# ChalmersPhotonicsLab/QAMpy

Hardware: AMD Instinct MI355X
Metric: equalised MSym/s (2-pol, 2 SPS) (higher is better)
Workload: dtype f32

## Files before the change

### qampy_amd/csrc/api.hip

```cpp
#include "common.h"
#include <stdlib.h>
#include <atomic>
#include <mutex>
#include <vector>
#include <unordered_map>
#include <string.h>

namespace qh {

thread_local hipStream_t g_stream = nullptr;
static thread_local hipStream_t g_streams[4] = {nullptr, nullptr, nullptr, nullptr};
int g_device = -1;
static thread_local std::string g_err;
static std::mutex g_mu;

void set_error(const std::string &s) { g_err = s; }

int hip_fail(hipError_t e, const char *what, const char *file, int line)
{
    g_err = std::string(hipGetErrorString(e)) + " in " + what + " (" + file + ":" + std::to_string(line) + ")";
    (void)hipGetLastError();
    return QH_ERR_HIP;
}

// ... 4 lines not shown
static int reserved_cus()
{
    int v = g_reserved_cus.load();
    if (v < 0) { const char *e = getenv("QAMPY_HIP_RESERVED_CUS"); v = e ? atoi(e) : 32; if (v < 0) v = 0; g_reserved_cus.store(v); }
    return v;
}
double gram_budget_gb()
{
    double v = g_gram_budget_gb.load();
    if (v < 0) { const char *e = getenv("QAMPY_HIP_GRAM_BUDGET_GB"); v = e ? atof(e) : 160.0; if (!(v > 0)) v = 160.0; g_gram_budget_gb.store(v); }
    return v;
}
static std::atomic<int> g_pit_timing{-1};
int pit_timing_mode()
{
    int v = g_pit_timing.load();
    if (v < 0) { const char *e = getenv("QAMPY_HIP_PIT_TIMING"); v = !e ? 1 : (e[0] == 'a' ? 2 : (e[0] == 'n' ? 0 : 1)); g_pit_timing.store(v); }
    return v;
}
int default_tier() { return g_default_tier.load(); }
double default_tier_tol() { return g_default_tol.load(); }

static int init_device(int device)
{
    std::lock_guard<std::mutex> lk(g_mu);
    if (g_stream && device == g_device) return QH_OK;
    if (g_device >= 0 && device != g_device) {
        set_error("libqampy_hip is already initialised on device " + std::to_string(g_device) + ": one device per process");
        return QH_ERR_ARG;
    }
    int n = 0;
    if (hipGetDeviceCount(&n) != hipSuccess || n <= 0) {
        (void)hipGetLastError();
        set_error("no HIP device visible: libqampy_hip needs a gfx950 (MI355X) GPU, there is no CPU fallback");
        return QH_ERR_NODEVICE;
    }
    if (device < 0 || device >= n) { set_error("device index out of range"); return QH_ERR_ARG; }
    hipDeviceProp_t prop;
    QH_HIP(hipGetDeviceProperties(&prop, device));
    if (strncmp(prop.gcnArchName, "gfx950", 6) != 0) {
        set_error(std::string("device is ") + prop.gcnArchName + ", libqampy_hip is built for gfx950 only");
        return QH_ERR_NODEVICE;
    }
    QH_HIP(hipSetDevice(device));
    int prio_least = 0, prio_greatest = 0;
    QH_HIP(hipDeviceGetStreamPriorityRange(&prio_least, &prio_greatest));
    for (int i = 0; i < 4; i++) {
        if (g_streams[i]) { (void)hipStreamDestroy(g_streams[i]); g_streams[i] = nullptr; }
        if (i == 2) {
            const int reserved = reserved_cus();
            const int ncu = prop.multiProcessorCount;
            if (reserved > 0 && reserved < ncu) {
                std::vector<uint32_t> mask((ncu + 31) / 32, 0u);
                for (int c = reserved; c < ncu; c++) mask[c / 32] |= 1u << (c % 32);
                if (hipExtStreamCreateWithCUMask(&g_streams[i], (uint32_t)mask.size(), mask.data()) == hipSuccess) continue;
                (void)hipGetLastError();
                g_streams[i] = nullptr;
            }
        }
        QH_HIP(hipStreamCreateWithPriority(&g_streams[i], hipStreamNonBlocking, i == 2 ? prio_least : prio_greatest));
    }
    g_stream = g_streams[0];
    g_device = device;
    return QH_OK;
}

hipStream_t side_stream() { return g_stream == g_streams[0] ? g_streams[1] : g_streams[0]; }
hipStream_t helper_stream() { return g_streams[3]; }

int ensure_init()
{
    if (g_stream) return QH_OK;
    return init_device(g_device >= 0 ? g_device : 0);
}

constexpr int SCRATCH_SLOTS = (int)Slot::COUNT;
thread_local void *g_scratch[SCRATCH_SLOTS] = {nullptr};
thread_local size_t g_scratch_n[SCRATCH_SLOTS] = {0};
thread_local unsigned g_scratch_epoch = 0;
static std::atomic<int> g_form[FORM_COUNT];
struct FormName { const char *key, *env; };
static const FormName FORM_NAMES[FORM_COUNT] = {
    {"trainer", "QAMPY_HIP_TRAINER"}, {"pit_form", "QAMPY_HIP_PIT_FORM"}, {"seg_lanes", "QAMPY_HIP_SEG_LANES"}, {"pit_probe", "QAMPY_HIP_PIT_PROBE"},
    {"bps", "QAMPY_HIP_BPS"}, {"pit_tail", "QAMPY_HIP_PIT_TAIL"}};
static int form_parse(int k, const char *v, int *out)
{
    if (!v || !v[0]) { *out = 0; return 0; }
    switch (k) {
    case FORM_TRAINER: *out = v[0] == 'd' ? 1 : (v[0] == 'l' ? 2 : (v[0] == 'i' ? 3 : (v[0] == 'a' || v[0] == '0' ? 0 : -1))); break;
    case FORM_PIT: *out = v[0] == 's' ? 1 : (v[0] == 'b' ? 2 : (v[0] == 'a' || v[0] == '0' ? 0 : -1)); break;
    case FORM_SEG_LANES: { const int n = atoi(v); *out = (n == 8 || n == 16 || n == 0) ? n : -1; break; }
    case FORM_BPS: *out = v[0] == 't' ? 1 : (v[0] == 'l' ? 2 : (v[0] == 'a' || v[0] == '0' ? 0 : -1)); break;
    case FORM_PIT_TAIL: *out = v[0] == 's' ? 1 : (v[0] == 'a' || v[0] == '0' ? 0 : -1); break;
    default: *out = atoi(v) != 0 ? 1 : 0; break;
    }
    return *out < 0 ? -1 : 0;
}
static const int g_form_env_read = [] {
    for (int k = 0; k < FORM_COUNT; k++) {
        int v = 0;
        if (form_parse(k, getenv(FORM_NAMES[k].env), &v) == 0) g_form[k].store(v);
    }
    return 0;
}();
int form(FormKey k) { return g_form[k].load(std::memory_order_relaxed); }
const char *trainer_force()
{
    switch (form(FORM_TRAINER)) {
    case 1: return "direct";
    case 2: return "lookahead";
    case 3: return "iterative";
    default: return "";
    }
}
static constexpr int POOL_CLASSES = 48, POOL_KEEP = 8;
static constexpr size_t POOL_BYTES = (size_t)24 << 30;
static std::vector<void *> g_pool[POOL_CLASSES];
static size_t g_pool_bytes = 0;
static void pool_release();
static int pool_class(size_t bytes) { int k = 8; while (((size_t)1 << k) < bytes && k < POOL_CLASSES - 1) k++; return k; }
int pool_alloc(size_t bytes, void **p, size_t *cap)
{
    const int k = pool_class(bytes);
    *cap = (size_t)1 << k;
    {
        std::lock_guard<std::mutex> lk(g_mu);
        if (!g_pool[k].empty()) { *p = g_pool[k].back(); g_pool[k].pop_back(); g_pool_bytes -= *cap; return QH_OK; }
    }
    hipError_t e = hipMalloc(p, *cap);
    if (e == hipErrorOutOfMemory) {
        (void)hipGetLastError();
        (void)hipDeviceSynchronize();
        pool_release();
        e = hipMalloc(p, *cap);
    }
    QH_HIP(e);
    return QH_OK;
}
void pool_free(void *p, size_t cap)
{
    const int k = pool_class(cap);
    {
        std::lock_guard<std::mutex> lk(g_mu);
        if ((int)g_pool[k].size() < POOL_KEEP && g_pool_bytes + cap <= POOL_BYTES) { g_pool[k].push_back(p); g_pool_bytes += cap; return; }
    }
    (void)hipFree(p);
}
static std::unordered_map<void *, size_t> g_dlive;
static void pool_release()
{
    std::lock_guard<std::mutex> lk(g_mu);
    for (auto &v : g_pool) { for (void *p : v) (void)hipFree(p); v.clear(); }
    g_pool_bytes = 0;
}

static std::vector<void *> g_hpool[POOL_CLASSES];
static size_t g_hpool_bytes = 0;
static constexpr size_t HPOOL_BYTES = (size_t)8 << 30;
static std::vector<std::pair<void *, size_t>> g_hlive;
int pinned_alloc(size_t bytes, void **p)
{
    const int k = pool_class(bytes ? bytes : 1);
    const size_t cap = (size_t)1 << k;
    {
        std::lock_guard<std::mutex> lk(g_mu);
        if (!g_hpool[k].empty()) { *p = g_hpool[k].back(); g_hpool[k].pop_back(); g_hpool_bytes -= cap; g_hlive.emplace_back(*p, cap); return QH_OK; }
    }
    QH_HIP(hipHostMalloc(p, cap, hipHostMallocDefault));
    std::lock_guard<std::mutex> lk(g_mu);
    g_hlive.emplace_back(*p, cap);
    return QH_OK;
}
int pinned_free(void *p)
{
    size_t cap = 0;
    {
// ... 311 lines not shown
```

### qampy_amd/csrc/common.h

```cpp
#pragma once
#include <hip/hip_runtime.h>
#include <stdint.h>
#include <string>
#include <vector>
#include "../../include/qampy_hip.h"

namespace qh {

extern thread_local hipStream_t g_stream;
extern int g_device;
void set_error(const std::string &s);
int hip_fail(hipError_t e, const char *what, const char *file, int line);

#define QH_HIP(call)                                                        \
    do {                                                                    \
        hipError_t _e = (call);                                             \
        if (_e != hipSuccess) return qh::hip_fail(_e, #call, __FILE__, __LINE__); \
    } while (0)

#define QH_REQUIRE(cond, msg)                                   \
    do {                                                        \
        if (!(cond)) { qh::set_error(msg); return QH_ERR_ARG; } \
    } while (0)

#define QH_WAVE_FIRST() __builtin_amdgcn_s_setprio(3)

int ensure_init();
hipStream_t side_stream();
hipStream_t helper_stream();
enum FormKey { FORM_TRAINER = 0, FORM_PIT, FORM_SEG_LANES, FORM_PIT_PROBE, FORM_BPS, FORM_PIT_TAIL, FORM_COUNT };
int form(FormKey k);
const char *trainer_force();
double gram_budget_gb();
int pit_timing_mode();
int default_tier();
double default_tier_tol();
enum class Slot : int {
    BPS_ANGLES,
    BPS_CHUNKS,
    BPS_ALPHABET,
    TWOSTAGE,
    STEP_SIZES,
    GRAM,
    BI_LEVELS,
    PIT_WORK,
    PIT_CTRL,
    PIT_COV,
    PIT_BASIS,
    PIT_ROTATIONS,
    PIT_ACQ,
    PIT_MODEL,
    SER,
    SYNTH,
    METRICS,
    SNR_EST,
    AWGN_MC,
    CD_TABLE,
    RESAMPLE_TABLE,
    ROW_MOMENTS,
    FOE,
    IMPAIR,
    PMD,
    TXRESP,
    SOS,
    CPR,
    FFT,
    IQ,
    SYNC,
    PEAK,
    PILOT,
    PRECOMP,
    BLIND,
    HYBRID,
    FIBRE,
    COUNT
};
int scratch(Slot slot, size_t bytes, void **p);
unsigned scratch_epoch();

struct TableCache {
    std::string key;
    std::vector<char> host;
    void *dev = nullptr;
    unsigned epoch = 0;
    template <typename F> int get(Slot slot, const std::string &k, size_t bytes, F fill, const void **tab)
    {
        void *p = nullptr;
        int rc;
        if (dev && key == k && epoch == scratch_epoch()) {
            if ((rc = scratch(slot, bytes, &p))) return rc;
            if (p == dev) { *tab = p; return QH_OK; }
        }
        if (dev) QH_HIP(hipDeviceSynchronize());
        dev = nullptr;
        if ((rc = scratch(slot, bytes, &p))) return rc;
        host.resize(bytes);
        fill(host.data());
        QH_HIP(hipMemcpyAsync(p, host.data(), bytes, hipMemcpyHostToDevice, g_stream));
        key = k; dev = p; epoch = scratch_epoch();
        *tab = p;
        return QH_OK;
    }
};
template <typename T> inline void key_add(std::string &k, const T &v) { k.append(reinterpret_cast<const char *>(&v), sizeof(T)); }

constexpr double QH_PI = 3.14159265358979323846, QH_TWO_PI = 2 * QH_PI;

inline size_t up256(size_t n) { return (n + 255) & ~(size_t)255; }
struct ScratchLayout {
    size_t total = 0;
    size_t take(size_t bytes) { const size_t o = total; total += up256(bytes); return o; }
};
template <typename K> int dyn_lds(K kernel, size_t bytes)
// ... 158 lines not shown
```

### qampy_amd/csrc/train_pit.h

```cpp
#pragma once
#include <atomic>
#include <chrono>
#include <vector>
#include "train_impl.h"
#include "train_seg.h"

namespace qh {

typedef qh_pit_report PitCtrl;

constexpr double PIT_CONTRACT = 0.2;
constexpr int PIT_PROBE = 128;
constexpr int PIT_SEEDWIN = 512;
constexpr int PIT_MAXSEG = 65536;

__host__ __device__ inline int pit_symmetry(int method)
{
    switch (method) {
    case QH_M_CMA: case QH_M_SGNCMA: case QH_M_RDE: return 0;
    case QH_M_CMA2: return 2;
    default: return 4;
    }
}

// ... 47 lines not shown
}

template <typename R>
__global__ void __launch_bounds__(256) pit_setup_kernel(const Cx<R> *E, int nmodes, int64_t L, int64_t npow, int ntot, const R *mu, double gear,
                                                        double bound, double tol, PitSeg sg, PitCtrl *c, R *mu_acq)
{
    QH_WAVE_FIRST();
    __shared__ double red[256];
    double acc = 0;
    for (int k = 0; k < nmodes; k++)
        for (int64_t i = threadIdx.x; i < npow; i += 256) {
            const Cx<R> v = E[(size_t)k * L + i];
            acc += (double)v.re * v.re + (double)v.im * v.im;
        }
    red[threadIdx.x] = acc;
    __syncthreads();
    for (int s = 128; s > 0; s >>= 1) {
        if (threadIdx.x < s) red[threadIdx.x] += red[threadIdx.x + s];
        __syncthreads();
    }
    if (threadIdx.x == 0) {
        const double p = red[0] / ((double)nmodes * (double)npow);
        const double m = (double)*mu;
        double ma = gear * m;
        const double cap = bound / ((double)ntot * (p > 1e-30 ? p : 1e-30));
        if (ma > cap) ma = cap;
        if (!(ma > m)) ma = m;
        c->segments = sg.S; c->seg_len = sg.len; c->mu = m; c->mu_acq = ma; c->power = p; c->tol = tol;
        for (int q = 0; q < QH_PIT_MAXPASS; q++) { c->result_change[q] = -1; c->deviation[q] = -1; c->deviation_rms[q] = -1; c->deviation_taps[q] = -1; c->deviation_taps_worst[q] = -1; } c->passes = 0; c->converged = 0; c->acq_chunks = 0; c->acq_steps = 0; c->acq_done = 0; c->done = 0; c->diverged = 0; c->corr_on = 0; c->gain = 0; c->out_power = 0;
        for (int i = 0; i < QH_PIT_MAXPASS; i++) c->defect[i] = -1;
        for (int i = 0; i < QH_PIT_MAXCHUNK; i++) c->acq_err[i] = -1;
        *mu_acq = (R)ma;
    }
}

template <typename R>
__global__ void __launch_bounds__(256) pit_acq_monitor_kernel(const Cx<R> *err, int64_t err_pitch, int64_t step0, int64_t n, int nsel,
                                                              const int64_t *modes_dev, double plateau, PitCtrl *c, R *mu_acq, const R *mu, double floor_gear)
{
    QH_WAVE_FIRST();
    if (threadIdx.x == 0 && floor_gear >= 0) {
        const R lo = (R)((double)*mu * floor_gear), h = *mu_acq * (R)0.5;
        *mu_acq = h > lo ? h : (*mu_acq > lo ? lo : *mu_acq);
    }
    if (c->acq_done) return;
    __shared__ double red[256];
    double acc = 0;
    for (int j = 0; j < nsel; j++) {
        const Cx<R> *row = err + (size_t)modes_dev[j] * err_pitch + step0;
        for (int64_t i = threadIdx.x; i < n; i += 256) {
            const Cx<R> v = row[i];
            acc += (double)v.re * v.re + (double)v.im * v.im;
        }
    }
    red[threadIdx.x] = acc;
    __syncthreads();
    for (int s = 128; s > 0; s >>= 1) {
        if (threadIdx.x < s) red[threadIdx.x] += red[threadIdx.x + s];
        __syncthreads();
    }
    if (threadIdx.x == 0) {
        const double v = red[0] / ((double)n * nsel);
        const int k = c->acq_chunks;
        if (k < QH_PIT_MAXCHUNK) c->acq_err[k] = v;
        c->acq_chunks = k + 1;
        c->acq_steps = step0 + n;
        if (!(v == v) || v > 1e30) { c->diverged = 1; c->acq_done = 1; return; }
        if (k >= 1) {
            const double prev = c->acq_err[k - 1 < QH_PIT_MAXCHUNK ? k - 1 : QH_PIT_MAXCHUNK - 1];
            if (v > 100 * c->acq_err[0]) { c->diverged = 1; c->acq_done = 1; return; }
            if (v > plateau * prev) c->acq_done = 1;
        }
    }
}

template <typename R> __global__ void pit_acq_finish_kernel(Cx<R> *wx, const Cx<R> *w_start, int n, PitCtrl *c)
{
    QH_WAVE_FIRST();
    const int i = blockIdx.x * blockDim.x + threadIdx.x;
    if (c->diverged && i < n) wx[i] = w_start[i];
}

inline size_t pit_phase_pitch(int ntaps, int os, int nwin) { return (size_t)nwin + (size_t)(ntaps + os - 1) / os + 1; }
template <typename R>
__global__ void __launch_bounds__(256) pit_phase_kernel(const Cx<R> *E, int nmodes, int64_t L, int os, const Cx<R> *wx, int ntaps, PitSeg sg,
                                                        const int64_t *modes_dev, int nwin, double *z)
{
    QH_WAVE_FIRST();
    extern __shared__ __attribute__((aligned(16))) char pit_smem[];
    Cx<R> *w = reinterpret_cast<Cx<R> *>(pit_smem);
    const int ntot = nmodes * ntaps;
    const int pitch = nwin + (ntaps + os - 1) / os + 1;
    Cx<R> *xs = w + ntot;
    __shared__ double rr[256], ri[256];
    const int s = blockIdx.x, j = blockIdx.y;
    const int mode = (int)modes_dev[j];
    for (int f = threadIdx.x; f < ntot; f += 256) w[f] = wx[(size_t)mode * ntot + f];
    const int64_t st = sg.start(s);
    int64_t n = sg.steps(s);
    if (n > nwin) n = nwin;
    const int ns = n > 0 ? (int)(n - 1) * os + ntaps : 0;
    for (int k = 0; k < nmodes; k++) {
        const Cx<R> *x = E + (size_t)k * L + st * os;
        for (int g = threadIdx.x; g < ns; g += 256) xs[((size_t)k * os + g % os) * pitch + g / os] = x[g];
    }
    __syncthreads();
    double zr = 0, zi = 0;
    for (int i = threadIdx.x; i < n; i += 256) {
        R yr = 0, yi = 0;
        for (int k = 0; k < nmodes; k++) {
            const Cx<R> *wk = w + k * ntaps;
            for (int r = 0; r < os; r++) {
                const Cx<R> *xp = xs + ((size_t)k * os + r) * pitch + i;
                int u = 0;
                for (int t = r; t < ntaps; t += os, u++) {
                    const Cx<R> a = xp[u], b = wk[t];
                    yr = fma_(a.re, b.re, fma_(-a.im, b.im, yr));
                    yi = fma_(a.re, b.im, fma_(a.im, b.re, yi));
                }
            }
        }
        const double y2r = (double)yr * yr - (double)yi * yi, y2i = 2.0 * yr * yi;
        zr += y2r * y2r - y2i * y2i;
        zi += 2.0 * y2r * y2i;
    }
    rr[threadIdx.x] = zr; ri[threadIdx.x] = zi;
    __syncthreads();
    for (int q = 128; q > 0; q >>= 1) {
        if (threadIdx.x < q) { rr[threadIdx.x] += rr[threadIdx.x + q]; ri[threadIdx.x] += ri[threadIdx.x + q]; }
        __syncthreads();
    }
    if (threadIdx.x == 0) { z[2 * ((size_t)s * gridDim.y + j)] = rr[0]; z[2 * ((size_t)s * gridDim.y + j) + 1] = ri[0]; }
}

static __global__ void __launch_bounds__(256) pit_unwrap_kernel(const double *z, int S, int nsel, double *rot, double *phi, int *jump)
{
    QH_WAVE_FIRST();
    __shared__ int ptot[512];
    const double q = 1.5707963267948966;
    phi += (size_t)blockIdx.x * S; jump += (size_t)blockIdx.x * S;
    for (int j = blockIdx.x; j <= (int)blockIdx.x; j++) {
        for (int s = threadIdx.x; s < S; s += 256) {
            const double zr = z[2 * ((size_t)s * nsel + j)], zi = z[2 * ((size_t)s * nsel + j) + 1];
            phi[s] = (zr == 0 && zi == 0) ? 0.0 : (double)atan2f((float)-zi, (float)-zr) / 4;
        }
        __syncthreads();
        for (int s = threadIdx.x; s < S; s += 256) jump[s] = s == 0 ? 0 : (int)rint((phi[s - 1] - phi[s]) / q);
        __syncthreads();
        block_prefix_sum<int>(jump, S, ptot);
        for (int s = threadIdx.x; s < S; s += 256) {
            const double p = phi[s] + q * (jump[s] & 3);
            float sn, cs;
            sincosf((float)p, &sn, &cs);
            rot[2 * ((size_t)s * nsel + j)] = cs;
            rot[2 * ((size_t)s * nsel + j) + 1] = -sn;
        }
        __syncthreads();
    }
}

template <typename R>
__global__ void __launch_bounds__(256) pit_seed_kernel(const Cx<R> *wx, int nmodes, int ntot, const int64_t *modes_dev, int nsel, const double *rot, Cx<R> *X,
                                                       const Cx<R> *w0, Cx<R> *Y, PitCtrl *c)
{
    QH_WAVE_FIRST();
    const int s = blockIdx.x;
    const int n = nmodes * ntot;
    if (s == 0 && c) {
        if (threadIdx.x == 0) { c->done = 0; c->converged = 0; c->passes = 0; }
        for (int q = threadIdx.x; q < QH_PIT_MAXPASS; q += 256) {
            c->result_change[q] = -1; c->deviation[q] = -1; c->deviation_rms[q] = -1; c->deviation_taps[q] = -1; c->deviation_taps_worst[q] = -1; c->defect[q] = -1;
        }
    }
    const bool exact0 = s == 0 && w0 != nullptr;
    for (int e = threadIdx.x; e < n; e += 256) {
        const int row = e / ntot;
        Cx<R> v = exact0 ? w0[e] : wx[e];
        if (rot && !exact0) {
            for (int j = 0; j < nsel; j++)
                if ((int)modes_dev[j] == row) {
                    const double c = rot[2 * ((size_t)s * nsel + j)], d = rot[2 * ((size_t)s * nsel + j) + 1];
                    const double vr = (double)v.re * c - (double)v.im * d, vi = (double)v.re * d + (double)v.im * c;
                    v = Cx<R>{(R)vr, (R)vi};
                    break;
                }
        }
        X[(size_t)s * n + e] = v;
        Y[(size_t)s * n + e] = v;
    }
}

template <typename R>
__global__ void __launch_bounds__(PIT_PROBE) pit_defect_kernel(const Cx<R> *E, int nmodes, int64_t L, int os, int ntaps, PitSeg sg, int64_t TrSyms,
                                                                const int64_t *modes_dev, const Cx<R> *X, const Cx<R> *Y, int sym, const PitCtrl *c, double *dfc, double *pw, double *gph,
                                                                const Cx<R> *wx_prev)
{
    QH_WAVE_FIRST();
    if (c->done) return;
    extern __shared__ __attribute__((aligned(16))) char pit_smem[];
    Cx<R> *wa = reinterpret_cast<Cx<R> *>(pit_smem);
    const int ntot = nmodes * ntaps;
    Cx<R> *wb = wa + ntot;
    const int pitch = PIT_PROBE + (ntaps + os - 1) / os + 1;
    Cx<R> *xs = wb + ntot;
    __shared__ double red[4][PIT_PROBE];
    const int b = blockIdx.x + 1, j = blockIdx.y;
    const int mode = (int)modes_dev[j];
    const size_t wset = (size_t)nmodes * ntot;
    const bool result_probe = b == sg.S;
    for (int f = threadIdx.x; f < ntot; f += PIT_PROBE) {
        wa[f] = result_probe ? wx_prev[(size_t)mode * ntot + f] : X[(size_t)b * wset + (size_t)mode * ntot + f];
        wb[f] = Y[(size_t)(b - 1) * wset + (size_t)mode * ntot + f];
    }
    const int64_t st0 = result_probe ? (TrSyms > PIT_PROBE ? TrSyms - PIT_PROBE : 0) : sg.start(b);
    int64_t nout = TrSyms - st0;
    if (nout > PIT_PROBE) nout = PIT_PROBE;
    const int ns = nout > 0 ? (int)(nout - 1) * os + ntaps : 0;
    for (int k = 0; k < nmodes; k++) {
        const Cx<R> *x = E + (size_t)k * L + st0 * os;
        for (int g = threadIdx.x; g < ns; g += PIT_PROBE) xs[((size_t)k * os + g % os) * pitch + g / os] = x[g];
    }
    __syncthreads();
    double aa = 0, bb = 0, cr = 0, ci = 0;
    if (threadIdx.x < nout) {
        R ar = 0, ai = 0, br = 0, bi = 0;
        for (int k = 0; k < nmodes; k++)
            for (int r = 0; r < os; r++) {
                const Cx<R> *xp = xs + ((size_t)k * os + r) * pitch + threadIdx.x;
                int u = 0;
                for (int t = r; t < ntaps; t += os, u++) {
                    const Cx<R> v = xp[u], p = wa[k * ntaps + t], q = wb[k * ntaps + t];
                    ar = fma_(v.re, p.re, fma_(-v.im, p.im, ar)); ai = fma_(v.re, p.im, fma_(v.im, p.re, ai));
                    br = fma_(v.re, q.re, fma_(-v.im, q.im, br)); bi = fma_(v.re, q.im, fma_(v.im, q.re, bi));
                }
            }
        aa = (double)ar * ar + (double)ai * ai;
        bb = (double)br * br + (double)bi * bi;
        cr = (double)br * ar + (double)bi * ai;
        ci = (double)bi * ar - (double)br * ai;
    }
// ... 1796 lines not shown
        if (exact_only) {
            QH_REQUIRE(!o.exchange, "train_equaliser: a capture split over processes needs the parallel-in-time solver (blind / decision-directed method, fixed step)");
            void *cb0 = nullptr;
            if ((rc = scratch(Slot::PIT_CTRL, sizeof(PitCtrl) + 64, &cb0))) return rc;
            PitCtrl *c0 = report_dev ? (PitCtrl *)report_dev : (PitCtrl *)cb0;
            PitSeg s1; s1.S = 1; s1.len = TrSyms; s1.extra = 0; s1.tail = 0;
            hipLaunchKernelGGL((pit_setup_kernel<R>), dim3(1), dim3(256), 0, g_stream, (const Cx<R> *)E, nmodes, L, (int64_t)(L < 4096 ? L : 4096), nmodes * ntaps, (const R *)mu_dev, 1.0, 1.0,
                               o.tol > 0 ? o.tol : 1e-3, s1, c0, (R *)((char *)cb0 + sizeof(PitCtrl)));
            return exact_form(c0, o.adaptive, zero_err, adaptive ? nullptr : gram, 0);
        }
    }
    if (adaptive) o.acquire = 0;
    const int ntot = nmodes * ntaps;
    const int npass = o.max_passes > 0 ? o.max_passes : (adaptive ? QH_PIT_MAXPASS : 16);
    const double tol = (o.tol > 0 ? o.tol : 1e-3) * (adaptive ? 1.0 / 3.0 : 1.0);
    const double safety = o.dev_safety > 0 ? o.dev_safety : PIT_DEV_SAFETY;
    const int sym = pit_symmetry(method);
    const bool seed_phase = o.phase_seed < 0 ? sym == 4 : o.phase_seed != 0;
    const bool want_corr = o.correction != 0 && pit_basis_ok(ntot, sizeof(Cx<R>));
    double beta = o.corr_beta >= 0 ? o.corr_beta : (sym == 0 ? 1.5 : 0.0);

    void *cbuf = nullptr;
    if ((rc = scratch(Slot::PIT_CTRL, sizeof(PitCtrl) + 64, &cbuf))) return rc;
    PitCtrl *ctrl = report_dev ? (PitCtrl *)report_dev : (PitCtrl *)cbuf;
    R *mu_acq = (R *)((char *)cbuf + sizeof(PitCtrl));

    int S = o.segments;
    const float ad_relax = 1.0f, ad_damp = 0.7f;
    const int ad_newton = 1;
    const int64_t head_want = 16384;
    int64_t head = adaptive ? ((TrSyms / 4 < head_want ? TrSyms / 4 : head_want) / LA_B * LA_B) : 0;
    if (!adaptive && o.head_steps > 0) {
        QH_REQUIRE(!o.exchange, "train_equaliser: a capture split over processes takes no exact head");
        head = (int64_t)o.head_steps / LA_B * LA_B;
        if (head > TrSyms) head = TrSyms / LA_B * LA_B;
        o.acquire = 0;
    }
    int64_t seg_want = 2048;
    if (adaptive && !(method == QH_M_SBD || method == QH_M_MDDMA || method == QH_M_DD)) {
        const int64_t t = ((TrSyms - head) / 512 + LA_B - 1) / LA_B * LA_B;
        if (t > seg_want) seg_want = t;
    }
    if (S == 0 && adaptive) S = (int)((TrSyms - head) / seg_want < PIT_MAXSEG ? (TrSyms - head) / seg_want : PIT_MAXSEG);
    if (S == 0) {
        R mu_h = (R)o.mu_hint;
        if (!(o.mu_hint > 0)) {
            QH_HIP(hipMemcpyAsync(&mu_h, mu_dev, sizeof(R), hipMemcpyDeviceToHost, g_stream));
            QH_HIP(hipStreamSynchronize(g_stream));
        }
        S = pit_auto_segments(TrSyms, (double)mu_h, nsel, o.acquire);
    }
    PitPlan pl = pit_plan(o, TrSyms, head, S, adaptive, o.acquire ? o.acq_chunk : 0);
    const PitSeg &sg = pl.sg;
    if (zero_err) QH_HIP(hipMemsetAsync(err, 0, (size_t)nmodes * TrSyms * Niter * sizeof(Cx<R>), g_stream));
    const int64_t npow = L < 4096 ? L : 4096;
    hipLaunchKernelGGL((pit_setup_kernel<R>), dim3(1), dim3(256), 0, g_stream, (const Cx<R> *)E, nmodes, L, npow, ntot, (const R *)mu_dev, pl.gear, pl.bound, tol, sg, ctrl, mu_acq);
    QH_HIP(hipGetLastError());
    if (TrSyms == 0 || Niter == 0) return QH_OK;
    if (sg.S < 2) {
        const double zero = 0;
        QH_HIP(hipMemcpyAsync(&ctrl->defect[0], &zero, sizeof(double), hipMemcpyHostToDevice, g_stream));
        return exact_form(ctrl, adaptive ? 1 : 0, 0, gram, 1);
    }

    TrainerForm f;
    if ((rc = trainer_form<R>(f, FORM_PASSES, method, adaptive, nmodes, ntaps, os, sg.len, (int64_t)sg.S * nsel, symbols, nsy, modes, nsel))) return rc;
    if (adaptive && !f.seg) return exact_form(ctrl, 1, 0, nullptr, 0);
    const bool decision = method == QH_M_SBD || method == QH_M_MDDMA || method == QH_M_DD;
    const bool seg_form = f.seg, use_bi = f.use_bi, block_form = f.block, pair_tab = f.pair_tab;
    const bool split = o.exchange != nullptr;
    const int own_first = split ? o.seg_first : 0, own_count = split ? o.seg_count : sg.S;
    const bool xchg_async = split && o.exchange_on_stream != 0;
    if (split) {
        QH_REQUIRE(seg_form, "train_equaliser: a capture split over processes needs the throughput form of the passes (>= 512 chains, supported tap layout)");
        QH_REQUIRE(own_first >= 0 && own_count >= 0 && own_first + own_count <= sg.S, "train_equaliser: owned segments outside the segment grid");
        QH_REQUIRE(Niter == 1, "train_equaliser: a capture split over processes is trained in one sweep");
    }

    const size_t wset = (size_t)nmodes * ntot;
    const size_t wbytes = wset * sizeof(Cx<R>);
    void *wbuf = nullptr;
    const size_t nsj = (size_t)sg.S * nsel;
    const size_t bytes_w = ((2 * (size_t)sg.S + 2) * wbytes + 63) / 64 * 64;
    if ((rc = scratch(Slot::PIT_WORK, bytes_w + 10 * nsj * sizeof(double) + (size_t)nsel * sizeof(int64_t) + 320 + nsj * 16 + 4 * ((nsj + 63) / 64) * sizeof(float) + 64, &wbuf))) return rc;
    Cx<R> *X = (Cx<R> *)wbuf, *Y = X + (size_t)sg.S * wset, *w_start = Y + (size_t)sg.S * wset, *w_call = w_start + wset;
    double *z = (double *)((char *)wbuf + bytes_w), *rot = z + 2 * nsj, *dfc = rot + 2 * nsj, *pw = dfc + nsj, *gph = pw + nsj, *theta = gph + 2 * nsj;
    int64_t *modes_dev = (int64_t *)(theta + 2 * nsj);
    double *uw_phi = (double *)(modes_dev + ((nsel + 7) / 8 * 8));
    int *uw_jump = (int *)(uw_phi + (size_t)sg.S * nsel);
    float *devmax = (float *)(uw_jump + (size_t)sg.S * nsel);
    const int ndev = (int)((nsj + 63) / 64);
    unsigned *ticket = (unsigned *)(devmax + 4 * (size_t)ndev);
    PitInit init{};
    init.z[0] = ticket; init.zn[0] = sizeof(unsigned);
    R *ad_rS = nullptr, *ad_rE = nullptr;
    Cx<R> *ad_eS = nullptr, *ad_eE = nullptr, *ad_errh = nullptr;
    float *ad_M = nullptr, *ad_chg = nullptr, *ad_rP = nullptr, *ad_dP = nullptr;
    if (!adaptive && head > 0) {
        void *ab = nullptr;
        if ((rc = scratch(Slot::PIT_ACQ, (size_t)nmodes * head * sizeof(Cx<R>) + 64, &ab))) return rc;
        ad_errh = (Cx<R> *)ab;
    }
    if (adaptive) {
        void *ab = nullptr;
        const size_t nS = ((size_t)sg.S + 15) / 16 * 16;
        if ((rc = scratch(Slot::PIT_ACQ, nS * (2 * sizeof(R) + 2 * sizeof(Cx<R>) + 3 * sizeof(float)) + 64 + (size_t)nmodes * head * sizeof(Cx<R>), &ab))) return rc;
        ad_eS = (Cx<R> *)ab; ad_eE = ad_eS + nS; ad_errh = ad_eE + nS;
        ad_rS = (R *)(ad_errh + (size_t)nmodes * head); ad_rE = ad_rS + nS;
        ad_M = (float *)(ad_rE + nS); ad_rP = ad_M + nS; ad_dP = ad_rP + nS; ad_chg = ad_dP + nS;
    }
    init.modes_dev = modes_dev; init.nsel = nsel;
    for (int j = 0; j < 16; j++) init.modes[j] = j < nsel ? modes[j] : 0;
    const bool prepared = o.prepared != nullptr && o.acquire && !adaptive && head == 0 && Niter >= 1;
    const bool need_mu = adaptive || !(o.mu_hint > 0), need_acq = o.acquire && !(o.acq_chunk > 0) && !prepared;
    R mu_acq_h = 0;
    if (need_acq) QH_HIP(hipMemcpyAsync(&mu_acq_h, mu_acq, sizeof(R), hipMemcpyDeviceToHost, g_stream));
    R mu_host = need_mu ? (R)1 : (R)o.mu_hint;
    if (need_mu) QH_HIP(hipMemcpyAsync(&mu_host, mu_dev, sizeof(R), hipMemcpyDeviceToHost, g_stream));
    if (need_mu || need_acq) QH_HIP(hipStreamSynchronize(g_stream));
    if (!adaptive && !(mu_host != 0))
        return exact_form(ctrl, 0, 0, gram, 0);
    if (o.acquire && !(o.acq_chunk > 0)) pl.acquisition(o, TrSyms, pit_acq_chunk(mu_acq_h));

    const int64_t amax = pl.amax;
    void *G = const_cast<void *>(gram);
    if (prepared) QH_REQUIRE(seg_form && o.acq_chunk > 0, "train_equaliser: a prepared acquisition belongs to throughput-form passes with acq_chunk given (qh_pit_prepare_*_dev said so)");
    if (block_form && !G && (!seg_form || amax > 0) && !prepared) {
        const int64_t n = seg_form ? pl.ngram : TrSyms;
        rc = pair_tab ? gram_build<R>(E, nmodes, L, os, ntaps, n, &G) : gram_cur_build<R>(E, nmodes, L, os, ntaps, n, &G);
        if (rc) return rc;
    }
    const int64_t g_per_step = pair_tab ? LA_B : GRAM_TRI / 2 / LA_B;

    const int ncol = sg.S * nsel;
    const double *lam = nullptr;
    const Zf *Vb = nullptr;
    Zf *Dz[2] = {nullptr, nullptr};
    Zf *Xe = nullptr, *Ye = nullptr, *Yprev = nullptr;
    if (want_corr) {
        void *cb = nullptr;
        if ((rc = scratch(Slot::PIT_BASIS, pit_basis_bytes(ntot) + 4 * (size_t)ntot * ncol * sizeof(Zf) + (size_t)ntot * nsel * sizeof(Zf) + 256, &cb))) return rc;
        void *basis = o.basis ? o.basis : cb;
        if (!o.basis && (rc = pit_basis<R>(E, nmodes, L, os, ntaps, TrSyms, basis))) return rc;
        lam = (const double *)basis; Vb = (const Zf *)((const char *)basis + (size_t)ntot * sizeof(double));
        Dz[0] = (Zf *)((char *)cb + (pit_basis_bytes(ntot) + 63) / 64 * 64); Dz[1] = Dz[0] + (size_t)ntot * ncol;
        Xe = Dz[1] + (size_t)ntot * ncol; Ye = Xe + (size_t)ntot * ncol; Yprev = Ye + (size_t)ntot * ncol;
    }
    const bool eig = want_corr && sizeof(R) == 4 && form(FORM_PIT_PROBE) == 0;
    const bool tail_fused = eig && seg_form && !adaptive && !split && form(FORM_PIT_TAIL) == 0;
    const bool tables_ok = method == QH_M_CMA || method == QH_M_SGNCMA || method == QH_M_MCMA || method == QH_M_RDE || method == QH_M_MRDE ||
                           (decision && (use_bi || seg_form));
    const bool ssb = eig && tables_ok && method != QH_M_CMA2;
    PitModel *model = nullptr;
    float4 *ualpha = nullptr;
    float2 *uqv = nullptr;
    PitModelArgs<R> ma;
    hipEvent_t model_event = nullptr;
    if (ssb) {
        void *mb = nullptr;
        const size_t pw_ = 2 * PIT_EIGMAX + 8;
        const size_t b_part = (size_t)PIT_MODB * 4 * nsel * pw_ * sizeof(float), b_u = ((size_t)nsel * ntot * sizeof(Cx<R>) + 63) / 64 * 64;
        const size_t b_ua = ((size_t)ncol * sizeof(float4) + 63) / 64 * 64, b_uq = ((size_t)ncol * sizeof(float2) + 63) / 64 * 64;
        if ((rc = scratch(Slot::PIT_MODEL, b_part + b_u + b_ua + b_uq + 16 * sizeof(PitModel) + 128, &mb))) return rc;
        ma.part = (float *)mb; ma.u = (Cx<R> *)((char *)mb + b_part);
        ualpha = (float4 *)((char *)mb + b_part + b_u); uqv = (float2 *)((char *)ualpha + b_ua);
        model = (PitModel *)((char *)uqv + b_uq); ma.model = model; ma.ticket = (unsigned *)(model + 16);
        init.z[1] = ma.ticket; init.zn[1] = sizeof(unsigned);
        init.z[2] = ualpha; init.zn[2] = (unsigned)(b_ua + b_uq);
        ma.E = (const Cx<R> *)E; ma.wx = (const Cx<R> *)wx; ma.L = L; ma.TrSyms = TrSyms; ma.nmodes = nmodes; ma.ntaps = ntaps; ma.os = os; ma.nsel = nsel; ma.method = method;
        if (decision) { ma.symbols = (const Cx<R> *)f.dd_table; ma.nsy = 2 * f.dd_npart + 1; ma.sy_pitch = 2 * BI_DD_MAXLEV; ma.tables = 1; }
        else { ma.symbols = (const Cx<R> *)symbols; ma.nsy = nsy; ma.sy_pitch = nsy; ma.tables = (method == QH_M_RDE || method == QH_M_MRDE) ? 1 : 0; }
        for (int j = 0; j < 16; j++) ma.modes[j] = j < nsel ? modes[j] : 0;
        if (o.corr_beta < 0) beta = 0.0;
    }
    const size_t glds = ((size_t)PIT_EIGMAX * PIT_EIGMAX + (size_t)PIT_EIGMAX * PIT_GT) * sizeof(Zf);
    static std::atomic<bool> gemm_attr{false};
    if (want_corr && !gemm_attr.load(std::memory_order_acquire)) {
        QH_HIP(hipFuncSetAttribute((const void *)pit_cgemm_kernel<R, true>, hipFuncAttributeMaxDynamicSharedMemorySize, 160 * 1024 - 256));
        QH_HIP(hipFuncSetAttribute((const void *)pit_cgemm_kernel<R, false>, hipFuncAttributeMaxDynamicSharedMemorySize, 160 * 1024 - 256));
        QH_HIP(hipFuncSetAttribute((const void *)pit_basis_mfma_kernel<R, 0>, hipFuncAttributeMaxDynamicSharedMemorySize, 128 * 1024));
        QH_HIP(hipFuncSetAttribute((const void *)pit_basis_mfma_kernel<R, 1>, hipFuncAttributeMaxDynamicSharedMemorySize, 128 * 1024));
        QH_HIP(hipFuncSetAttribute((const void *)pit_tail_kernel<R>, hipFuncAttributeMaxDynamicSharedMemorySize, 128 * 1024));
        gemm_attr.store(true, std::memory_order_release);
    }

    LaArgs<R> la = la_args<R>(E, L, nmodes, ntaps, os, modes, nsel, method, symbols, nsy, mu_dev, err, TrSyms * Niter);
    la.G = (const GramPair<R> *)G; la.gpair = pair_tab ? 1 : 0; la.wx_cs = (int64_t)wset;
    la.dd_general = f.dd_general;
    f.alphabet(la);
    const TrainArgs<R> ta = train_args<R>(E, L, nmodes, ntaps, os, TrSyms, Niter, modes, nsel, method, symbols, nsy, mu_dev, err);

    PitTiming &tm = pit_timing();
    tm.npass = 0; tm.acq_ms = 0;
    bool acq_timed = false;
    PitEvents &ev = pit_events();
    QH_REQUIRE(ev.ok, "train_equaliser: no pinned memory for the pass flags");
    const bool redo_ok = o.exact_redo_off == 0;
    bool fell_back = false;
    if (redo_ok && !adaptive) { init.cd[0] = w_call; init.cs[0] = wx; init.cn[0] = (unsigned)wbytes; }
    if (o.acquire && Niter > 0) { init.cd[1] = w_start; init.cs[1] = wx; init.cn[1] = (unsigned)wbytes; }
    hipLaunchKernelGGL(pit_init_kernel, dim3(32), dim3(256), 0, g_stream, init);
    QH_HIP(hipGetLastError());
    for (int it = 0; it < Niter; it++) {
        if (it == 0 && prepared) {
            const PitPrepLayout lay = pit_prep_layout<R>(nmodes, ntaps, amax);
            const char *pb = (const char *)o.prepared;
            hipLaunchKernelGGL((pit_adopt_kernel<R>), dim3((unsigned)((wset + 255) / 256)), dim3(256), 0, g_stream, (Cx<R> *)wx, (const Cx<R> *)(pb + lay.wx), (int)wset,
                               (const PitCtrl *)(pb + lay.ctrl), ctrl, mu_acq, (const R *)(pb + lay.mu_acq));
            QH_HIP(hipGetLastError());
        } else if (it == 0 && o.acquire) {
            if (pl.nchunks > 0) { QH_HIP(hipEventRecord(ev.t0[PIT_NEV - 1], g_stream)); acq_timed = true; }
            if ((rc = pit_acq_enqueue<R>(pl, block_form ? &la : nullptr, use_bi, &ta, (Cx<R> *)wx, (Cx<R> *)err, TrSyms * Niter, ctrl, mu_acq, mu_dev,
                                         modes_dev, nsel))) return rc;
            if (pl.nchunks > 0) QH_HIP(hipEventRecord(ev.t1[PIT_NEV - 1], g_stream));
            hipLaunchKernelGGL((pit_acq_finish_kernel<R>), dim3((unsigned)((wset + 255) / 256)), dim3(256), 0, g_stream, (Cx<R> *)wx, (const Cx<R> *)w_start, (int)wset, ctrl);
            QH_HIP(hipGetLastError());
        }
        if (adaptive) {
            QH_HIP(hipMemcpyAsync(w_start, wx, wbytes, hipMemcpyDeviceToDevice, g_stream));
            QH_HIP(hipMemcpyAsync(ad_chg + 1, mu_dev, sizeof(R), hipMemcpyDeviceToDevice, g_stream));
            if ((rc = train_dev<R>(E, nmodes, L, head, 1, os, mu_dev, wx, ntaps, modes, 1, 1, symbols, nsy, method, ad_errh, 0, nullptr))) return rc;
            QH_HIP(hipMemcpyAsync((Cx<R> *)err + (size_t)modes[0] * TrSyms, ad_errh + (size_t)modes[0] * head, (size_t)head * sizeof(Cx<R>), hipMemcpyDeviceToDevice, g_stream));
            hipLaunchKernelGGL((pit_adapt_init_kernel<R>), dim3((sg.S + 255) / 256), dim3(256), 0, g_stream, (const R *)mu_dev, (const Cx<R> *)(ad_errh + (size_t)modes[0] * head + head - 1),
                               sg.S, ad_rS, ad_eS);
            QH_HIP(hipGetLastError());
        }
        if (!adaptive && head > 0) {
            if ((rc = train_dev<R>(E, nmodes, L, head, 1, os, mu_dev, wx, ntaps, modes, nsel, 0, symbols, nsy, method, ad_errh, 0, nullptr))) return rc;
            for (int j = 0; j < nsel; j++)
                QH_HIP(hipMemcpyAsync((Cx<R> *)err + (size_t)modes[j] * TrSyms * Niter + (size_t)it * TrSyms, ad_errh + (size_t)modes[j] * head, (size_t)head * sizeof(Cx<R>),
                                      hipMemcpyDeviceToDevice, g_stream));
        }
        const double *rot_use = nullptr;
        if (seed_phase) {
            int nwin = PIT_SEEDWIN;
            auto phase_lds = [&](int nw) { return ((size_t)ntot + (size_t)nmodes * os * pit_phase_pitch(ntaps, os, nw)) * sizeof(Cx<R>); };
            while (nwin > 32 && phase_lds(nwin) > 60 * 1024) nwin /= 2;
            QH_REQUIRE(phase_lds(nwin) <= 60 * 1024, "train_equaliser: phase seeding does not fit the LDS for this filter shape (pass phase_seed = 0)");
            hipLaunchKernelGGL((pit_phase_kernel<R>), dim3(sg.S, nsel), dim3(256), phase_lds(nwin), g_stream, (const Cx<R> *)E, nmodes, L, os,
                               (const Cx<R> *)wx, ntaps, sg, (const int64_t *)modes_dev, nwin, z);
            hipLaunchKernelGGL(pit_unwrap_kernel, dim3(nsel), dim3(256), 0, g_stream, (const double *)z, sg.S, nsel, rot, uw_phi, uw_jump);
            rot_use = rot;
        }
        const Cx<R> *w_exact = o.start == 1 ? nullptr : ((it == 0 && o.acquire) ? (const Cx<R> *)w_start : (const Cx<R> *)wx);
        hipLaunchKernelGGL((pit_seed_kernel<R>), dim3(sg.S), dim3(256), 0, g_stream, (const Cx<R> *)wx, nmodes, ntot, (const int64_t *)modes_dev, nsel, rot_use, X, w_exact, Y, ctrl);
        if (ssb) {
            ma.sg = sg; ma.rot = rot_use;
            static thread_local hipEvent_t ev_seed = nullptr, ev_model = nullptr;
            if (!ev_seed) { QH_HIP(hipEventCreateWithFlags(&ev_seed, hipEventDisableTiming)); QH_HIP(hipEventCreateWithFlags(&ev_model, hipEventDisableTiming)); }
            hipStream_t ss = helper_stream();
            QH_HIP(hipEventRecord(ev_seed, g_stream));
            QH_HIP(hipStreamWaitEvent(ss, ev_seed, 0));
            hipLaunchKernelGGL((pit_model_kernel<R, 0>), dim3(PIT_MODB), dim3(256), 0, ss, ma);
            hipLaunchKernelGGL((pit_model_kernel<R, 1>), dim3(PIT_MODB), dim3(256), 0, ss, ma);
            QH_HIP(hipEventRecord(ev_model, ss));
            model_event = ev_model;
        }
        QH_HIP(hipGetLastError());
        const int timing_mode = pit_timing_mode();
        auto decide_args = [&](int p, const float *dm, const float2 *ye, float2 *yprev, int ne, int ncol_e, int corr_wanted) {
            PitDecideArgs<R> d;
            d.dfc = dfc; d.pw = pw; d.nb = (int)((sg.S - 1) * nsel); d.Ylast = (const Cx<R> *)(Y + (size_t)(sg.S - 1) * wset); d.n = (int)wset; d.wx = (Cx<R> *)wx; d.c = ctrl;
            d.host_view = &ev.hview[2 * p]; d.nrow = nsel; d.devmax = dm; d.ndev = ndev; d.safety = safety; d.Ye = ye; d.Yprev = yprev; d.ne = ne; d.ncol_e = ncol_e;
            d.theta = theta; d.modes_dev = (const int64_t *)modes_dev; d.ntot_w = ntot; d.S = (int)sg.S; d.sym = sym; d.corr_wanted = corr_wanted;
            d.extra = adaptive ? (const float *)ad_chg : nullptr;
            d.Dfin = (ye && !adaptive) ? (const float2 *)Dz[1] : nullptr; d.Vfin = (const float2 *)Vb; d.lam_fin = lam;
            d.stall_from = o.correction == 0 ? QH_PIT_MAXPASS : (adaptive ? 5 : 2);
            return d;
        };
        auto timed = [&](int p) { return timing_mode == 2 || (timing_mode == 1 && p == 1); };
        int back_done_for = 0;
        auto enqueue_pass = [&](int p) -> int {
            ((volatile float *)ev.hview)[2 * p] = -1.f;
            PitFuse<R> fz;
            fz.X = X; fz.Y = Y; fz.theta = theta; fz.modes_dev = (const int64_t *)modes_dev; fz.nmodes = nmodes; fz.nsel = nsel;
            fz.damp = (adaptive && p > 1) ? ad_damp : 1.f;
            fz.x_only = tail_fused ? 1 : 0;
            if (p > 0 && tail_fused && back_done_for == p) {
            } else if (p > 0 && want_corr) {
                if (eig)
                    hipLaunchKernelGGL((pit_basis_mfma_kernel<R, 1>), dim3((ncol + PIT_MC - 1) / PIT_MC), dim3(pit_mfma_threads(ntot)), pit_mfma_lds(ntot), g_stream, Vb + (size_t)ntot * ntot,
                                       (const Cx<R> *)nullptr, (const Zf *)Dz[1], (Zf *)nullptr, ntot, ncol, (const PitCtrl *)ctrl, fz);
                else
                    hipLaunchKernelGGL((pit_cgemm_kernel<R, false>), dim3((ncol + PIT_GT - 1) / PIT_GT), dim3(256), glds, g_stream, Vb + (size_t)ntot * ntot, (const Zf *)Dz[1], (Zf *)nullptr, ntot, ncol, (const PitCtrl *)ctrl, fz);
                QH_HIP(hipGetLastError());
            } else if (p > 0) {
                QH_HIP(hipMemcpyAsync(X + wset, Y, (size_t)(sg.S - 1) * wbytes, hipMemcpyDeviceToDevice, g_stream));
                QH_HIP(hipMemcpyAsync(Y, X, (size_t)sg.S * wbytes, hipMemcpyDeviceToDevice, g_stream));
            }
            if (o.on_pass) {
                hipStream_t keep = g_stream;
                o.on_pass(o.on_pass_user, it, p);
                g_stream = keep;
            }
            if (timed(p)) QH_HIP(hipEventRecord(ev.t0[p], g_stream));
            if (seg_form) {
                SegArgs<R> sa{};
                sa.E = (const Cx<R> *)E; sa.wx = tail_fused ? X : Y; sa.wx_out = tail_fused ? Y : nullptr; sa.symbols = la.symbols; sa.err = (Cx<R> *)err; sa.mu = mu_dev;
                sa.L = L; sa.TrSyms = TrSyms; sa.nsy = la.nsy; sa.sy_pitch = la.sy_pitch; sa.err_pitch = TrSyms * Niter; sa.err_off = (int64_t)it * TrSyms;
                sa.nmodes = nmodes; sa.ntaps = ntaps; sa.os = os; sa.nsel = nsel; sa.S = sg.S;
                sa.seg_len = sg.len; sa.seg_extra = sg.extra; sa.seg_tail = sg.tail; sa.seg_begin = sg.begin;
                sa.r_in = ad_rS; sa.r_out = ad_rE; sa.e_in = ad_eS; sa.e_out = ad_eE; sa.mu_sum = (R *)ad_M; sa.adapt_first = sg.begin > 0 ? 1 : 0;
                for (int j = 0; j < 16; j++) sa.modes[j] = j < nsel ? modes[j] : 0;
                sa.skip = &ctrl->done;
                sa.q_first = own_first * nsel; sa.q_count = split ? own_count * nsel : 0;
                pit_last_launch().form = 1;
                if (!split || own_count > 0) { int r = launch_seg<R>(sa, method, adaptive); if (r) return r; }
                if (adaptive) hipLaunchKernelGGL((pit_adapt_scan_kernel<R>), dim3(1), dim3(1024), 0, g_stream, ad_rS, (const R *)ad_rE, ad_eS, (const Cx<R> *)ad_eE, sg.S, ad_chg, (const PitCtrl *)ctrl, ad_relax, ad_rP, ad_dP, ad_newton);
            } else if (block_form) {
                LaArgs<R> ls = la;
                ls.TrSyms = sg.len; ls.nch = sg.S; ls.wx = Y; ls.err_off = (int64_t)it * TrSyms; ls.seg = 1; ls.seg_extra = sg.extra; ls.seg_tail = sg.tail;
                ls.skip = &ctrl->done;
                pit_last_launch() = PitLaunch{use_bi ? 2 : 3, 0, 0, 0, 0, 0};
                if (sg.begin > 0) {
                    ls.E = (const Cx<R> *)E + sg.begin * os; ls.L = L - sg.begin * os; ls.err_off += sg.begin;
                    ls.G = (const GramPair<R> *)G + sg.begin * g_per_step;
                }
                { int r = use_bi ? launch_bi<R>(ls) : launch_la<R>(ls); if (r) return r; }
            } else {
                TrainArgs<R> ts = ta;
                ts.wx = Y; ts.nseg = sg.S; ts.seg_begin = sg.begin; ts.seg_len = sg.len; ts.seg_extra = sg.extra; ts.seg_tail = sg.tail; ts.seg_iter = it; ts.skip = &ctrl->done;
                pit_last_launch() = PitLaunch{4, 0, 0, 0, 0, 0};
                { int r = launch_any<R>(ts); if (r) return r; }
            }
// ... 218 lines not shown
```

Measured before the change: 1236.

## Fuse PIT phase seeding and unwrap into one kernel across modes

Adds a fused phase-seeding kernel that loads each segment's samples into LDS once and computes the fourth-power phase statistic for all selected modes (up to two) together. Each thread handles two output positions, with a 4-way unrolled, packed-float2 FMA inner loop. A last-block ticket then performs the phase unwrap and rotation computation in the same launch, replacing the separate unwrap kernel. This removes one launch, the duplicate sample loads per mode and the per-mode grid dimension. The cost is a serial per-thread scan over segments in the final block and a dependence on atomic ticket ordering.

```diff
diff --git a/qampy_amd/csrc/api.hip b/qampy_amd/csrc/api.hip
--- a/qampy_amd/csrc/api.hip
+++ b/qampy_amd/csrc/api.hip
@@ -110,7 +110,7 @@
 struct FormName { const char *key, *env; };
 static const FormName FORM_NAMES[FORM_COUNT] = {
     {"trainer", "QAMPY_HIP_TRAINER"}, {"pit_form", "QAMPY_HIP_PIT_FORM"}, {"seg_lanes", "QAMPY_HIP_SEG_LANES"}, {"pit_probe", "QAMPY_HIP_PIT_PROBE"},
-    {"bps", "QAMPY_HIP_BPS"}, {"pit_tail", "QAMPY_HIP_PIT_TAIL"}};
+    {"bps", "QAMPY_HIP_BPS"}, {"pit_tail", "QAMPY_HIP_PIT_TAIL"}, {"pit_phase", "QAMPY_HIP_PIT_PHASE"}};
 static int form_parse(int k, const char *v, int *out)
 {
     if (!v || !v[0]) { *out = 0; return 0; }
@@ -119,7 +119,7 @@
     case FORM_PIT: *out = v[0] == 's' ? 1 : (v[0] == 'b' ? 2 : (v[0] == 'a' || v[0] == '0' ? 0 : -1)); break;
     case FORM_SEG_LANES: { const int n = atoi(v); *out = (n == 8 || n == 16 || n == 0) ? n : -1; break; }
     case FORM_BPS: *out = v[0] == 't' ? 1 : (v[0] == 'l' ? 2 : (v[0] == 'a' || v[0] == '0' ? 0 : -1)); break;
-    case FORM_PIT_TAIL: *out = v[0] == 's' ? 1 : (v[0] == 'a' || v[0] == '0' ? 0 : -1); break;
+    case FORM_PIT_TAIL: case FORM_PIT_PHASE: *out = v[0] == 's' ? 1 : (v[0] == 'a' || v[0] == '0' ? 0 : -1); break;
     default: *out = atoi(v) != 0 ? 1 : 0; break;
     }
     return *out < 0 ? -1 : 0;
diff --git a/qampy_amd/csrc/common.h b/qampy_amd/csrc/common.h
--- a/qampy_amd/csrc/common.h
+++ b/qampy_amd/csrc/common.h
@@ -28,7 +28,7 @@
 int ensure_init();
 hipStream_t side_stream();
 hipStream_t helper_stream();
-enum FormKey { FORM_TRAINER = 0, FORM_PIT, FORM_SEG_LANES, FORM_PIT_PROBE, FORM_BPS, FORM_PIT_TAIL, FORM_COUNT };
+enum FormKey { FORM_TRAINER = 0, FORM_PIT, FORM_SEG_LANES, FORM_PIT_PROBE, FORM_BPS, FORM_PIT_TAIL, FORM_PIT_PHASE, FORM_COUNT };
 int form(FormKey k);
 const char *trainer_force();
 double gram_budget_gb();
diff --git a/qampy_amd/csrc/train_pit.h b/qampy_amd/csrc/train_pit.h
--- a/qampy_amd/csrc/train_pit.h
+++ b/qampy_amd/csrc/train_pit.h
@@ -153,6 +153,26 @@
 }
 
 inline size_t pit_phase_pitch(int ntaps, int os, int nwin) { return (size_t)nwin + (size_t)(ntaps + os - 1) / os + 1; }
+template <typename R> __device__ __forceinline__ void pit_phase_pow4(R yr, R yi, double &zr, double &zi)
+{
+    const double y2r = (double)yr * yr - (double)yi * yi, y2i = 2.0 * yr * yi;
+    zr += y2r * y2r - y2i * y2i;
+    zi += 2.0 * y2r * y2i;
+}
+constexpr double PIT_QUARTER = 1.5707963267948966;
+__device__ __forceinline__ double pit_seed_phi(double zr, double zi)
+{
+    return (zr == 0 && zi == 0) ? 0.0 : (double)atan2f((float)-zi, (float)-zr) / 4;
+}
+__device__ __forceinline__ int pit_seed_jump(double phi_prev, double phi) { return (int)rint((phi_prev - phi) / PIT_QUARTER); }
+__device__ __forceinline__ void pit_seed_rot(double phi, int jumps, double *rot)
+{
+    const double p = phi + PIT_QUARTER * (jumps & 3);
+    float sn, cs;
+    sincosf((float)p, &sn, &cs);
+    rot[0] = cs;
+    rot[1] = -sn;
+}
 template <typename R>
 __global__ void __launch_bounds__(256) pit_phase_kernel(const Cx<R> *E, int nmodes, int64_t L, int os, const Cx<R> *wx, int ntaps, PitSeg sg,
                                                         const int64_t *modes_dev, int nwin, double *z)
@@ -191,9 +211,7 @@
                 }
             }
         }
-        const double y2r = (double)yr * yr - (double)yi * yi, y2i = 2.0 * yr * yi;
-        zr += y2r * y2r - y2i * y2i;
-        zi += 2.0 * y2r * y2i;
+        pit_phase_pow4(yr, yi, zr, zi);
     }
     rr[threadIdx.x] = zr; ri[threadIdx.x] = zi;
     __syncthreads();
@@ -208,25 +226,144 @@
 {
     QH_WAVE_FIRST();
     __shared__ int ptot[512];
-    const double q = 1.5707963267948966;
     phi += (size_t)blockIdx.x * S; jump += (size_t)blockIdx.x * S;
     for (int j = blockIdx.x; j <= (int)blockIdx.x; j++) {
-        for (int s = threadIdx.x; s < S; s += 256) {
-            const double zr = z[2 * ((size_t)s * nsel + j)], zi = z[2 * ((size_t)s * nsel + j) + 1];
-            phi[s] = (zr == 0 && zi == 0) ? 0.0 : (double)atan2f((float)-zi, (float)-zr) / 4;
-        }
+        for (int s = threadIdx.x; s < S; s += 256) phi[s] = pit_seed_phi(z[2 * ((size_t)s * nsel + j)], z[2 * ((size_t)s * nsel + j) + 1]);
         __syncthreads();
-        for (int s = threadIdx.x; s < S; s += 256) jump[s] = s == 0 ? 0 : (int)rint((phi[s - 1] - phi[s]) / q);
+        for (int s = threadIdx.x; s < S; s += 256) jump[s] = s == 0 ? 0 : pit_seed_jump(phi[s - 1], phi[s]);
         __syncthreads();
         block_prefix_sum<int>(jump, S, ptot);
-        for (int s = threadIdx.x; s < S; s += 256) {
-            const double p = phi[s] + q * (jump[s] & 3);
-            float sn, cs;
-            sincosf((float)p, &sn, &cs);
-            rot[2 * ((size_t)s * nsel + j)] = cs;
-            rot[2 * ((size_t)s * nsel + j) + 1] = -sn;
-        }
+        for (int s = threadIdx.x; s < S; s += 256) pit_seed_rot(phi[s], jump[s], rot + 2 * ((size_t)s * nsel + j));
         __syncthreads();
+    }
+}
+
+constexpr int PIT_PHASE_SMAX = 4096;
+typedef float pit_f2 __attribute__((ext_vector_type(2)));
+template <typename R> struct PitMac {
+    R yr = 0, yi = 0;
+    __device__ __forceinline__ void mac(Cx<R> a, Cx<R> b) { yr = fma_(a.re, b.re, fma_(-a.im, b.im, yr)); yi = fma_(a.re, b.im, fma_(a.im, b.re, yi)); }
+    __device__ __forceinline__ R re() const { return yr; }
+    __device__ __forceinline__ R im() const { return yi; }
+};
+template <> struct PitMac<float> {
+    pit_f2 y = {0.f, 0.f};
+    __device__ __forceinline__ void mac(Cx<float> a, Cx<float> b)
+    {
+        y = __builtin_elementwise_fma(pit_f2{a.re, a.re}, pit_f2{b.re, b.im}, __builtin_elementwise_fma(pit_f2{a.im, a.im}, pit_f2{-b.im, b.re}, y));
+    }
+    __device__ __forceinline__ float re() const { return y.x; }
+    __device__ __forceinline__ float im() const { return y.y; }
+};
+__device__ __forceinline__ double pit_ld_agent(const double *p) { return __hip_atomic_load(p, __ATOMIC_RELAXED, __HIP_MEMORY_SCOPE_AGENT); }
+template <typename R, int NSEL>
+__global__ void __launch_bounds__(256) pit_phase_all_kernel(const Cx<R> *__restrict__ E, int nmodes, int64_t L, int os, const Cx<R> *__restrict__ wx, int ntaps, PitSeg sg,
+                                                            const int64_t *__restrict__ modes_dev, int nwin, double *z, double *rot, unsigned *ticket)
+{
+    QH_WAVE_FIRST();
+    extern __shared__ __attribute__((aligned(16))) char pit_smem[];
+    Cx<R> *xs = reinterpret_cast<Cx<R> *>(pit_smem);
+    const int ntot = nmodes * ntaps;
+    const int pitch = nwin + (ntaps + os - 1) / os + 1;
+    __shared__ double rr[256], ri[256];
+    __shared__ int ptot[4];
+    __shared__ int last;
+    const int s = blockIdx.x, S = gridDim.x;
+    const Cx<R> *wj[NSEL];
+#pragma unroll
+    for (int j = 0; j < NSEL; j++) wj[j] = wx + (size_t)modes_dev[j] * ntot;
+    const int64_t st = sg.start(s);
+    int64_t n = sg.steps(s);
+    if (n > nwin) n = nwin;
+    const int ns = n > 0 ? (int)(n - 1) * os + ntaps : 0;
+    for (int k = 0; k < nmodes; k++) {
+        const Cx<R> *x = E + (size_t)k * L + st * os;
+        for (int g = threadIdx.x; g < ns; g += 256) xs[((size_t)k * os + g % os) * pitch + g / os] = x[g];
+    }
+    __syncthreads();
+    double zr[NSEL], zi[NSEL];
+#pragma unroll
+    for (int j = 0; j < NSEL; j++) { zr[j] = 0; zi[j] = 0; }
+    for (int i0 = threadIdx.x; i0 < n; i0 += 512) {
+        const bool two = i0 + 256 < n;
+        const int i1 = two ? i0 + 256 : i0;
+        PitMac<R> acc[2][NSEL];
+        for (int k = 0; k < nmodes; k++) {
+            for (int r = 0; r < os; r++) {
+                const Cx<R> *xp = xs + ((size_t)k * os + r) * pitch;
+                int u = 0, t = r;
+                for (; t + 3 * os < ntaps; t += 4 * os, u += 4) {
+                    Cx<R> b[4][NSEL], a0[4], a1[4];
+#pragma unroll
+                    for (int v = 0; v < 4; v++) {
+#pragma unroll
+                        for (int j = 0; j < NSEL; j++) b[v][j] = wj[j][k * ntaps + t + v * os];
+                        a0[v] = xp[i0 + u + v]; a1[v] = xp[i1 + u + v];
+                    }
+#pragma unroll
+                    for (int v = 0; v < 4; v++)
+#pragma unroll
+                        for (int j = 0; j < NSEL; j++) {
+                            acc[0][j].mac(a0[v], b[v][j]);
+                            acc[1][j].mac(a1[v], b[v][j]);
+                        }
+                }
+                for (; t < ntaps; t += os, u++) {
+                    const Cx<R> a0 = xp[i0 + u], a1 = xp[i1 + u];
+#pragma unroll
+                    for (int j = 0; j < NSEL; j++) {
+                        const Cx<R> b = wj[j][k * ntaps + t];
+                        acc[0][j].mac(a0, b);
+                        acc[1][j].mac(a1, b);
+                    }
+                }
+            }
+        }
+#pragma unroll
+        for (int j = 0; j < NSEL; j++) {
+            pit_phase_pow4(acc[0][j].re(), acc[0][j].im(), zr[j], zi[j]);
+            if (two) pit_phase_pow4(acc[1][j].re(), acc[1][j].im(), zr[j], zi[j]);
+        }
+    }
+#pragma unroll
+    for (int j = 0; j < NSEL; j++) {
+        rr[threadIdx.x] = zr[j]; ri[threadIdx.x] = zi[j];
+        __syncthreads();
+        for (int q = 128; q > 0; q >>= 1) {
+            if (threadIdx.x < q) { rr[threadIdx.x] += rr[threadIdx.x + q]; ri[threadIdx.x] += ri[threadIdx.x + q]; }
+            __syncthreads();
+        }
+        if (threadIdx.x == 0) { z[2 * ((size_t)s * NSEL + j)] = rr[0]; z[2 * ((size_t)s * NSEL + j) + 1] = ri[0]; }
+        __syncthreads();
+    }
+    if (threadIdx.x == 0) {
+        __threadfence();
+        const unsigned t = atomicAdd(ticket, 1u);
+        last = t == (unsigned)S - 1;
+        if (last) { *ticket = 0; __threadfence(); }
+    }
+    __syncthreads();
+    if (!last) return;
+    const int len = (S + 255) / 256;
+    const int s0 = threadIdx.x * len, s1 = s0 + len < S ? s0 + len : S;
+    auto phi = [&](int e, int j) { return pit_seed_phi(pit_ld_agent(z + 2 * ((size_t)e * NSEL + j)), pit_ld_agent(z + 2 * ((size_t)e * NSEL + j) + 1)); };
+    for (int j = 0; j < NSEL; j++) {
+        const double before = (s0 > 0 && s0 < s1) ? phi(s0 - 1, j) : 0.0;
+        int loc = 0;
+        double prev = before;
+        for (int e = s0; e < s1; e++) {
+            const double cur = phi(e, j);
+            if (e > 0) loc += pit_seed_jump(prev, cur);
+            prev = cur;
+        }
+        int run = block_scan_excl<int>(loc, [](int x, int y) { return x + y; }, 0, ptot);
+        prev = before;
+        for (int e = s0; e < s1; e++) {
+            const double cur = phi(e, j);
+            if (e > 0) run += pit_seed_jump(prev, cur);
+            pit_seed_rot(cur, run, rot + 2 * ((size_t)e * NSEL + j));
+            prev = cur;
+        }
     }
 }
 
@@ -2189,7 +2326,7 @@
     void *wbuf = nullptr;
     const size_t nsj = (size_t)sg.S * nsel;
     const size_t bytes_w = ((2 * (size_t)sg.S + 2) * wbytes + 63) / 64 * 64;
-    if ((rc = scratch(Slot::PIT_WORK, bytes_w + 10 * nsj * sizeof(double) + (size_t)nsel * sizeof(int64_t) + 320 + nsj * 16 + 4 * ((nsj + 63) / 64) * sizeof(float) + 64, &wbuf))) return rc;
+    if ((rc = scratch(Slot::PIT_WORK, bytes_w + 10 * nsj * sizeof(double) + (size_t)nsel * sizeof(int64_t) + 320 + nsj * 16 + 4 * ((nsj + 63) / 64) * sizeof(float) + 2 * sizeof(unsigned) + 64, &wbuf))) return rc;
     Cx<R> *X = (Cx<R> *)wbuf, *Y = X + (size_t)sg.S * wset, *w_start = Y + (size_t)sg.S * wset, *w_call = w_start + wset;
     double *z = (double *)((char *)wbuf + bytes_w), *rot = z + 2 * nsj, *dfc = rot + 2 * nsj, *pw = dfc + nsj, *gph = pw + nsj, *theta = gph + 2 * nsj;
     int64_t *modes_dev = (int64_t *)(theta + 2 * nsj);
@@ -2199,7 +2336,7 @@
     const int ndev = (int)((nsj + 63) / 64);
     unsigned *ticket = (unsigned *)(devmax + 4 * (size_t)ndev);
     PitInit init{};
-    init.z[0] = ticket; init.zn[0] = sizeof(unsigned);
+    init.z[0] = ticket; init.zn[0] = 2 * sizeof(unsigned);
     R *ad_rS = nullptr, *ad_rE = nullptr;
     Cx<R> *ad_eS = nullptr, *ad_eE = nullptr, *ad_errh = nullptr;
     float *ad_M = nullptr, *ad_chg = nullptr, *ad_rP = nullptr, *ad_dP = nullptr;
@@ -2344,9 +2481,19 @@
             auto phase_lds = [&](int nw) { return ((size_t)ntot + (size_t)nmodes * os * pit_phase_pitch(ntaps, os, nw)) * sizeof(Cx<R>); };
             while (nwin > 32 && phase_lds(nwin) > 60 * 1024) nwin /= 2;
             QH_REQUIRE(phase_lds(nwin) <= 60 * 1024, "train_equaliser: phase seeding does not fit the LDS for this filter shape (pass phase_seed = 0)");
+            const size_t all_lds = (size_t)nmodes * os * pit_phase_pitch(ntaps, os, nwin) * sizeof(Cx<R>);
+            if (form(FORM_PIT_PHASE) == 0 && nsel <= 2 && sg.S <= PIT_PHASE_SMAX && all_lds <= 64 * 1024) {
+                if (nsel == 2)
+                    hipLaunchKernelGGL((pit_phase_all_kernel<R, 2>), dim3(sg.S), dim3(256), all_lds, g_stream, (const Cx<R> *)E, nmodes, L, os,
+                                       (const Cx<R> *)wx, ntaps, sg, (const int64_t *)modes_dev, nwin, z, rot, ticket + 1);
+                else
+                    hipLaunchKernelGGL((pit_phase_all_kernel<R, 1>), dim3(sg.S), dim3(256), all_lds, g_stream, (const Cx<R> *)E, nmodes, L, os,
+                                       (const Cx<R> *)wx, ntaps, sg, (const int64_t *)modes_dev, nwin, z, rot, ticket + 1);
+            } else {
             hipLaunchKernelGGL((pit_phase_kernel<R>), dim3(sg.S, nsel), dim3(256), phase_lds(nwin), g_stream, (const Cx<R> *)E, nmodes, L, os,
                                (const Cx<R> *)wx, ntaps, sg, (const int64_t *)modes_dev, nwin, z);
             hipLaunchKernelGGL(pit_unwrap_kernel, dim3(nsel), dim3(256), 0, g_stream, (const double *)z, sg.S, nsel, rot, uw_phi, uw_jump);
+            }
             rot_use = rot;
         }
         const Cx<R> *w_exact = o.start == 1 ? nullptr : ((it == 0 && o.acquire) ? (const Cx<R> *)w_start : (const Cx<R> *)wx);
```

New measurement: 1225. No clear change (-0.9%).
